# shendurelab/MIPGEN

Measured on AMD Instinct MI355X. Metric: candidate MIPs scored/sec (SVR), higher is better.
Workload: dtype f64

## Files before the change

### mipgen_amd/csrc/kernels_svr.hip

```cpp
#include <hip/hip_runtime.h>
#include "kernels.h"
#include "device_utils.h"
#include "exp2_coef.h"
#include "mip_record.h"
#include <stdlib.h>

namespace {

__device__ __forceinline__ void exp2x3(double& t0, double& t1, double& t2)
{
    constexpr double C[11] = EXP2_COEF_10;
    const double MAGIC = 6755399441055744.0;
    double m0, m1, m2, f0, f1, f2;
    const double cd = C[10];
    asm volatile(
        "v_add_f64 %[m0], %[t0], %[magic]\n\t"
        "v_add_f64 %[m1], %[t1], %[magic]\n\t"
        "v_add_f64 %[m2], %[t2], %[magic]\n\t"
        "v_add_f64 %[f0], %[m0], -%[magic]\n\t"
        "v_add_f64 %[f1], %[m1], -%[magic]\n\t"
        "v_add_f64 %[f2], %[m2], -%[magic]\n\t"
        "v_add_f64 %[f0], %[t0], -%[f0]\n\t"
        "v_add_f64 %[f1], %[t1], -%[f1]\n\t"
        "v_add_f64 %[f2], %[t2], -%[f2]\n\t"
        "v_fma_f64 %[t0], %[cd], %[f0], %[c9]\n\t"
        "v_fma_f64 %[t1], %[cd], %[f1], %[c9]\n\t"
        "v_fma_f64 %[t2], %[cd], %[f2], %[c9]\n\t"
        "v_fma_f64 %[t0], %[t0], %[f0], %[c8]\n\t"
        "v_fma_f64 %[t1], %[t1], %[f1], %[c8]\n\t"
        "v_fma_f64 %[t2], %[t2], %[f2], %[c8]\n\t"
        "v_fma_f64 %[t0], %[t0], %[f0], %[c7]\n\t"
        "v_fma_f64 %[t1], %[t1], %[f1], %[c7]\n\t"
        "v_fma_f64 %[t2], %[t2], %[f2], %[c7]\n\t"
        "v_fma_f64 %[t0], %[t0], %[f0], %[c6]\n\t"
        "v_fma_f64 %[t1], %[t1], %[f1], %[c6]\n\t"
        "v_fma_f64 %[t2], %[t2], %[f2], %[c6]\n\t"
        "v_fma_f64 %[t0], %[t0], %[f0], %[c5]\n\t"
        "v_fma_f64 %[t1], %[t1], %[f1], %[c5]\n\t"
        "v_fma_f64 %[t2], %[t2], %[f2], %[c5]\n\t"
        "v_fma_f64 %[t0], %[t0], %[f0], %[c4]\n\t"
        "v_fma_f64 %[t1], %[t1], %[f1], %[c4]\n\t"
        "v_fma_f64 %[t2], %[t2], %[f2], %[c4]\n\t"
        "v_fma_f64 %[t0], %[t0], %[f0], %[c3]\n\t"
        "v_fma_f64 %[t1], %[t1], %[f1], %[c3]\n\t"
        "v_fma_f64 %[t2], %[t2], %[f2], %[c3]\n\t"
        "v_fma_f64 %[t0], %[t0], %[f0], %[c2]\n\t"
        "v_fma_f64 %[t1], %[t1], %[f1], %[c2]\n\t"
        "v_fma_f64 %[t2], %[t2], %[f2], %[c2]\n\t"
        "v_fma_f64 %[t0], %[t0], %[f0], %[c1]\n\t"
        "v_fma_f64 %[t1], %[t1], %[f1], %[c1]\n\t"
        "v_fma_f64 %[t2], %[t2], %[f2], %[c1]\n\t"
        "v_fma_f64 %[t0], %[t0], %[f0], %[c0]\n\t"
        "v_fma_f64 %[t1], %[t1], %[f1], %[c0]\n\t"
        "v_fma_f64 %[t2], %[t2], %[f2], %[c0]\n\t"
        : [t0] "+v"(t0), [t1] "+v"(t1), [t2] "+v"(t2), [m0] "=&v"(m0), [m1] "=&v"(m1), [m2] "=&v"(m2),
          [f0] "=&v"(f0), [f1] "=&v"(f1), [f2] "=&v"(f2)
        : [cd] "v"(cd), [magic] "s"(MAGIC), [c0] "s"(C[0]), [c1] "s"(C[1]), [c2] "s"(C[2]), [c3] "s"(C[3]), [c4] "s"(C[4]),
          [c5] "s"(C[5]), [c6] "s"(C[6]), [c7] "s"(C[7]), [c8] "s"(C[8]), [c9] "s"(C[9]));
    t0 = __hiloint2double(__double2hiint(t0) + (__double2loint(m0) << 20), __double2loint(t0));
    t1 = __hiloint2double(__double2hiint(t1) + (__double2loint(m1) << 20), __double2loint(t1));
    t2 = __hiloint2double(__double2hiint(t2) + (__double2loint(m2) << 20), __double2loint(t2));
}

template <int N>
__device__ __forceinline__ double dpp_row_shr(double x)
{
    const int lo = __builtin_amdgcn_update_dpp(0, __double2loint(x), 0x110 | N, 0xf, 0xf, true);
    const int hi = __builtin_amdgcn_update_dpp(0, __double2hiint(x), 0x110 | N, 0xf, 0xf, true);
    return __hiloint2double(hi, lo);
}
__device__ __forceinline__ double readlane_f64(double x, int l)
{
    return __hiloint2double(__builtin_amdgcn_readlane(__double2hiint(x), l), __builtin_amdgcn_readlane(__double2loint(x), l));
}

__device__ __forceinline__ int arm_feat(int base, int idx) { return base + idx + (idx >= 15); }
__device__ __forceinline__ int ins_feat(int idx) { return F_INS + idx + (idx >= 63); }

}

extern "C" int mipgen_svr_scores_fit_lds(int np, int kc, int n_pairs, int ss_range, int ssmax, int Lmax, int n_arm, int group, int n_e, int n_l, int n_threads, int it_pitch)
{
    const SvrLayout La = svr_layout(np, ssmax - ss_range + 1, ssmax, Lmax, n_arm, group, n_e, n_l, n_threads, it_pitch);
    const SvrLayout Lb = svr_layout(np, ssmax - ss_range + 1, ssmax, Lmax, n_arm, group, n_l, n_e, n_threads, it_pitch);
    const int need = np * kc * n_pairs;
    return need <= La.total_bytes / 8 - La.pf && need <= Lb.total_bytes / 8 - Lb.pf;
}

extern "C" size_t mipgen_svr_lds_bytes_tile(int np, int ss_range, int ssmax, int Lmax, int n_arm, int group, int n_e, int n_l, int n_threads, int it_pitch)
{
    const SvrLayout La = svr_layout(np, ssmax - ss_range + 1, ssmax, Lmax, n_arm, group, n_e, n_l, n_threads, it_pitch);
    const SvrLayout Lb = svr_layout(np, ssmax - ss_range + 1, ssmax, Lmax, n_arm, group, n_l, n_e, n_threads, it_pitch);
    if ((size_t)La.tb_stride * group * 8 > 65535 || (size_t)Lb.tb_stride * group * 8 > 65535) return (size_t)1 << 30;
    const size_t a = (size_t)La.total_bytes, b = (size_t)Lb.total_bytes;
    return a > b ? a : b;
}

__device__ __forceinline__ void svr_steps2(double& a0, double& a1, uint32_t lu, uint32_t ld, uint32_t pg0, uint32_t pg1,
                                           double i00, double i01, double i02, double i10, double i11, double i12)
{
    double u00, u01, u02, d00, d01, d02, u10, u11, u12, d10, d11, d12;
    uint32_t au0, ad0, au1, ad1, s0, s1, s2, s3;
    asm volatile(
        "s_and_b32 %[s0], %[pg0], 0xffff\n\t"
        "s_lshr_b32 %[s1], %[pg0], 16\n\t"
        "s_and_b32 %[s2], %[pg1], 0xffff\n\t"
        "s_lshr_b32 %[s3], %[pg1], 16\n\t"
        "v_add_u32 %[au0], %[s0], %[lu]\n\t"
        "v_add_u32 %[ad0], %[s1], %[ld]\n\t"
        "v_add_u32 %[au1], %[s2], %[lu]\n\t"
        "v_add_u32 %[ad1], %[s3], %[ld]\n\t"
        "ds_read_b64 %[u00], %[au0]\n\t"
        "ds_read_b64 %[d00], %[ad0]\n\t"
        "ds_read_b64 %[u01], %[au0] offset:8\n\t"
        "ds_read_b64 %[d01], %[ad0] offset:8\n\t"
        "ds_read_b64 %[u02], %[au0] offset:16\n\t"
        "ds_read_b64 %[d02], %[ad0] offset:16\n\t"
        "ds_read_b64 %[u10], %[au1]\n\t"
        "ds_read_b64 %[d10], %[ad1]\n\t"
        "ds_read_b64 %[u11], %[au1] offset:8\n\t"
        "ds_read_b64 %[d11], %[ad1] offset:8\n\t"
        "ds_read_b64 %[u12], %[au1] offset:16\n\t"
        "ds_read_b64 %[d12], %[ad1] offset:16\n\t"
        "s_waitcnt lgkmcnt(10)\n\t"
        "v_mul_f64 %[u00], %[u00], %[d00]\n\t"
        "s_waitcnt lgkmcnt(8)\n\t"
        "v_mul_f64 %[u01], %[u01], %[d01]\n\t"
        "v_fma_f64 %[a0], %[i00], %[u00], %[a0]\n\t"
        "s_waitcnt lgkmcnt(6)\n\t"
        "v_mul_f64 %[u02], %[u02], %[d02]\n\t"
        "v_fma_f64 %[a0], %[i01], %[u01], %[a0]\n\t"
        "s_waitcnt lgkmcnt(4)\n\t"
        "v_mul_f64 %[u10], %[u10], %[d10]\n\t"
        "v_fma_f64 %[a0], %[i02], %[u02], %[a0]\n\t"
        "s_waitcnt lgkmcnt(2)\n\t"
        "v_mul_f64 %[u11], %[u11], %[d11]\n\t"
        "v_fma_f64 %[a1], %[i10], %[u10], %[a1]\n\t"
        "s_waitcnt lgkmcnt(0)\n\t"
        "v_mul_f64 %[u12], %[u12], %[d12]\n\t"
        "v_fma_f64 %[a1], %[i11], %[u11], %[a1]\n\t"
        "v_fma_f64 %[a1], %[i12], %[u12], %[a1]\n\t"
        : [a0] "+v"(a0), [a1] "+v"(a1), [u00] "=&v"(u00), [u01] "=&v"(u01), [u02] "=&v"(u02), [d00] "=&v"(d00), [d01] "=&v"(d01),
          [d02] "=&v"(d02), [u10] "=&v"(u10), [u11] "=&v"(u11), [u12] "=&v"(u12), [d10] "=&v"(d10), [d11] "=&v"(d11), [d12] "=&v"(d12),
          [au0] "=&v"(au0), [ad0] "=&v"(ad0), [au1] "=&v"(au1), [ad1] "=&v"(ad1), [s0] "=&s"(s0), [s1] "=&s"(s1), [s2] "=&s"(s2), [s3] "=&s"(s3)
        : [lu] "v"(lu), [ld] "v"(ld), [pg0] "s"(pg0), [pg1] "s"(pg1), [i00] "v"(i00), [i01] "v"(i01), [i02] "v"(i02),
          [i10] "v"(i10), [i11] "v"(i11), [i12] "v"(i12)
        : "memory", "scc");
}
__device__ __forceinline__ void svr_steps1(double& a0, uint32_t lu, uint32_t ld, uint32_t pg0, double i00, double i01, double i02)
{
    double u00, u01, u02, d00, d01, d02;
    uint32_t au0, ad0, s0, s1;
    asm volatile(
        "s_and_b32 %[s0], %[pg0], 0xffff\n\t"
        "s_lshr_b32 %[s1], %[pg0], 16\n\t"
        "v_add_u32 %[au0], %[s0], %[lu]\n\t"
        "v_add_u32 %[ad0], %[s1], %[ld]\n\t"
        "ds_read_b64 %[u00], %[au0]\n\t"
        "ds_read_b64 %[d00], %[ad0]\n\t"
        "ds_read_b64 %[u01], %[au0] offset:8\n\t"
        "ds_read_b64 %[d01], %[ad0] offset:8\n\t"
        "ds_read_b64 %[u02], %[au0] offset:16\n\t"
        "ds_read_b64 %[d02], %[ad0] offset:16\n\t"
        "s_waitcnt lgkmcnt(4)\n\t"
        "v_mul_f64 %[u00], %[u00], %[d00]\n\t"
        "s_waitcnt lgkmcnt(2)\n\t"
        "v_mul_f64 %[u01], %[u01], %[d01]\n\t"
        "v_fma_f64 %[a0], %[i00], %[u00], %[a0]\n\t"
        "s_waitcnt lgkmcnt(0)\n\t"
        "v_mul_f64 %[u02], %[u02], %[d02]\n\t"
        "v_fma_f64 %[a0], %[i01], %[u01], %[a0]\n\t"
        "v_fma_f64 %[a0], %[i02], %[u02], %[a0]\n\t"
        : [a0] "+v"(a0), [u00] "=&v"(u00), [u01] "=&v"(u01), [u02] "=&v"(u02), [d00] "=&v"(d00), [d01] "=&v"(d01), [d02] "=&v"(d02),
          [au0] "=&v"(au0), [ad0] "=&v"(ad0), [s0] "=&s"(s0), [s1] "=&s"(s1)
        : [lu] "v"(lu), [ld] "v"(ld), [pg0] "s"(pg0), [i00] "v"(i00), [i01] "v"(i01), [i02] "v"(i02)
        : "memory", "scc");
}

template <int C>
__device__ __forceinline__ void svr_scan_rows(const __attribute__((address_space(3))) uint32_t* tab,
                                              const __attribute__((address_space(3))) double* sv,
                                              __attribute__((address_space(3))) double* out, bool act, double c2)
{
    typedef __attribute__((address_space(3))) const char lds_cc;
    typedef __attribute__((address_space(3))) const double lds_cd;
    lds_cc* svb = (lds_cc*)sv;
    double v[C];
    double tot = 0.0;
#pragma unroll
    for (int q = 0; q < C; q += 4) {
        uint32_t t[4];
        double g[4];
#pragma unroll
        for (int j = 0; j < 4; j++) if (q + j < C) t[j] = tab[q + j];
#pragma unroll
        for (int j = 0; j < 4; j++) if (q + j < C) g[j] = *(lds_cd*)(svb + t[j]);
#pragma unroll
        for (int j = 0; j < 4; j++) if (q + j < C) { v[q + j] = tot; tot = fma(g[j], c2, tot); }
    }
    double x = tot;
    x += dpp_row_shr<1>(x); x += dpp_row_shr<2>(x); x += dpp_row_shr<4>(x); x += dpp_row_shr<8>(x);
    const double base = x - tot;
    if (act) {
#pragma unroll
        for (int q = 0; q < C; q++) out[q * SVR_GROUP] = base + v[q];
    }
}

struct ScanDesc {
    int o0;
    int k;
    int ax, ay;
    int thr;
    int base;
    int len;
    int out;
    int ixo;
    int c;
    int blk;
    int pad[5];
};

#ifndef SVR_MIN_WAVES
#define SVR_MIN_WAVES 3
#endif
template <int CL>
__global__ __launch_bounds__(SVR_MAX_THREADS, 4) void k_svr_dense(
    const DevParams* __restrict__ P, const SvrGeom G, const DevRegion* __restrict__ regions,
    const SvrTile* __restrict__ tiles, int n_tiles, const uint8_t* __restrict__ bases,
    const int32_t* __restrict__ copy, const double* __restrict__ log10_tab, const double* __restrict__ model_all, int n_sv_all,
    double gamma_l2e, double rho, double s_guard, const uint64_t* __restrict__ records, double* __restrict__ scores,
    int n_split, double* __restrict__ partials, int64_t part_stride
#ifdef MIPGEN_DIAG
    , int dbg, unsigned long long* __restrict__ prof
#endif
    )
{
#ifndef MIPGEN_DIAG
    constexpr int dbg = 0;
    unsigned long long* const prof = nullptr;
#endif
    extern __shared__ __align__(16) unsigned char smem[];
    const unsigned long long blk_enter = ((dbg & 8) && prof) ? __builtin_amdgcn_s_memrealtime() : 0;
    const int unit = blockIdx.x;
    const int tile_i = unit / n_split, part = unit - tile_i * n_split;
    const SvrTile tile = tiles[tile_i];
    const DevRegion& R = regions[tile.region];
    const int groups_all = (n_sv_all + SVR_GROUP - 1) / SVR_GROUP, gpp = (groups_all + n_split - 1) / n_split;
    const int sv0 = part * gpp * SVR_GROUP;
    const double* __restrict__ model = model_all + (int64_t)sv0 * SV_ROW;
    const int n_sv = max(0, min(n_sv_all - sv0, gpp * SVR_GROUP));
    const int tid = threadIdx.x, lane = tid & (WAVE - 1);
    const int wid = __builtin_amdgcn_readfirstlane(tid / WAVE);
    const int NT = blockDim.x, NW = NT / WAVE;
    const bool minus = tile.strand != 0;

    const int A = P->n_pairs;
    const int Lmax = max(P->e_max, P->l_max);
    const int n_arm = max(G.n_e, G.n_l) | 1;
    const int Cmax_t = P->max_capture - (R.k0 + tile.ki0) * P->inc;
    const int Cmin_t = Cmax_t - (tile.kc - 1) * P->inc;
    const int ssmax = Cmax_t - P->min_sum, ssmin = Cmin_t - P->max_sum;
    const int p_first = R.first_pos + tile.p0;
    const int lo = p_first - Lmax;
    const int up_min = minus ? +P->l_min : +P->e_min;
    const int dn_min = minus ? +P->e_min : +P->l_min;
    const int n_up = minus ? +G.n_l : +G.n_e, n_dn = minus ? +G.n_e : +G.n_l;
    const int up_base = minus ? F_LIG : F_EXT, dn_base = minus ? F_EXT : F_LIG;
    const int up_len_f = minus ? F_LIG_LEN : F_EXT_LEN, dn_len_f = minus ? F_EXT_LEN : F_LIG_LEN;
    const int up_cp_f = minus ? F_LLC : F_LEC, dn_cp_f = minus ? F_LEC : F_LLC;
    const int up_norm_f = minus ? SVR_N_LIG : SVR_N_EXT, dn_norm_f = minus ? SVR_N_EXT : SVR_N_LIG;

    const SvrLayout L = svr_layout(tile.np, ssmin, ssmax, Lmax, n_arm, SVR_GROUP, n_up, n_dn, (int)blockDim.x, tile.pad >> 8);
    int L_ku = L.ku, L_kd = L.kd, L_tu = L.tu, L_td = L.td, L_ins = L.ins_len, L_up = L.up_cnt, L_dn = L.dn_cnt;
    asm volatile("" : "+s"(L_ku), "+s"(L_kd), "+s"(L_tu), "+s"(L_td), "+s"(L_ins), "+s"(L_up), "+s"(L_dn));
    const int S_ins = __builtin_amdgcn_readfirstlane(L.ins_sl), S_up = __builtin_amdgcn_readfirstlane(L.up_sl), S_dn = __builtin_amdgcn_readfirstlane(L.dn_sl);
    double* const dbase = (double*)smem;
    double* rinv = dbase + L.rinv;
    double* lg10 = dbase + L.lg10;
    uint32_t* ent_a = (uint32_t*)(smem + L.bytes_ent);
    uint32_t* ent_b = ent_a + L.n_ent_lds;
    const double cneg = -gamma_l2e, c2 = 2.0 * gamma_l2e;
    uint16_t* psum = (uint16_t*)(smem + L.bytes_psum);
    uint32_t* work = (uint32_t*)(smem + L.bytes_psum + 2 * SVR_MAX_CHUNK * (SVR_MAX_THREADS / 64));
    double* rows = dbase + L.rows;
    double* pfb = dbase + L.pf;
    double* tbb = dbase + L.tb;
    double* itb = dbase + L.it;
    ScanDesc* desc = (ScanDesc*)(smem + L.bytes_desc);
    uint32_t* sidx = (uint32_t*)(smem + L.bytes_idx);
    uint8_t* sb = smem + L.bytes_sb;
    const int ssr = ssmax - ssmin + 1;
    const int nq_t = L.nq;

    for (int i = tid; i < L.span_b + 8; i += NT) {
        int ri = lo + i - R.seq_start;
        sb[i] = (i < L.span_b && ri >= 0 && ri < R.seq_len) ? (bases[R.seq_off + ri] & BASE_CODE_MASK) : (uint8_t)BASE_OTHER;
    }
    for (int i = tid; i < L.rinv_len; i += NT) {
        rinv[3 * i] = i > 0 ? 1.0 / (double)i : 0.0; rinv[3 * i + 1] = i > 1 ? 1.0 / (double)(i - 1) : 0.0;
        rinv[3 * i + 2] = i > 2 ? 1.0 / (double)(i - 2) : 0.0;
    }
    for (int i = tid; i < 102; i += NT) lg10[i] = i == 0 ? 0.0 : (i <= 100 ? log10_tab[i] : 2.0);
    for (int i = tid; i < MIPGEN_N_LRC; i += NT) lg10[102 + i] = R.lrc[i];
    for (int i = tid; i < A && i < SVR_MAX_CHUNK * (SVR_MAX_THREADS / 64); i += NT) psum[i] = (uint16_t)((P->arm_ext[i] + P->arm_lig[i]) * L.it_p);
    if (tid < SVR_N_ARR) {
        ScanDesc d;
        const int k = tid;
        const bool ins = k < 3, up = k == 3 || k == 4;
        d.o0 = ins ? Lmax : (up ? 0 : Lmax + ssmin);
        d.k = ins ? k + 1 : ((k - 3) & 1) + 1;
        d.ax = ins ? 21 : 5; d.ay = ins ? 5 : 1; d.thr = ins ? 63 : 15;
        d.base = ins ? F_INS : (up ? up_base : dn_base);
        d.len = ins ? L_ins : (up ? L_up : L_dn);
        d.out = (ins ? k : 3) * S_ins + (ins ? 0 : (up ? k - 3 : 2)) * S_up + (k < 5 ? 0 : k - 5) * S_dn;
        d.ixo = d.out; d.c = (ins ? +S_ins : (up ? +S_up : +S_dn)) / 16;
        d.blk = ins ? 1 : ((up ? minus : !minus) ? 2 : 0);
        desc[k] = d;
    }
    __syncthreads();

    for (int k = 0; k < SVR_N_ARR; k++) {
        const ScanDesc d = desc[k];
        for (int i = tid; i < 16 * d.c; i += NT) {
            int slot = SVR_ZERO;
            if (i < d.len) {
                const int b0 = sb[d.o0 + i], b1 = sb[d.o0 + i + 1], b2 = sb[d.o0 + i + 2];
                const int last = d.k == 1 ? b0 : (d.k == 2 ? b1 : b2);
                const bool ok = b0 < 4 && (d.k < 2 || b1 < 4) && (d.k < 3 || b2 < 4);
                const int x = minus ? 3 - last : b0;
                const int y = d.k == 2 ? (minus ? 3 - b0 : b1) : (minus ? 3 - b1 : b1);
                const int z = minus ? 3 - b0 : b2;
                const int idx = d.ax * x + (d.k >= 2 ? d.ay * y + 1 : 0) + (d.k == 3 ? z + 1 : 0);
                if (ok) slot = d.k == 1 ? SVR_C1 + 4 * d.blk + x
                                        : d.base + idx + (idx >= d.thr);
            }
            sidx[d.ixo + i] = (uint32_t)(slot * (SVR_GROUP * 8));
        }
    }

    const int nU = tile.np * n_up, nD = nq_t * n_dn, n_ent = nU + nD;
    auto arm_entry = [&](int w, uint32_t& e_a, uint32_t& e_b, double* norm) __attribute__((always_inline)) {
        const bool up = w < nU;
        int wl, li, len, s;
        if (up) { wl = w / n_up; li = w - wl * n_up; len = up_min + li; s = Lmax + wl - len; }
        else { const int w2 = w - nU; wl = w2 / n_dn; li = w2 - wl * n_dn; len = dn_min + li; s = Lmax + ssmin + wl; }
        const bool is_lig = up ? minus : !minus;
        (void)norm;
        int cp = 1;
        if (R.copy_off >= 0) {
            const int slot = P->len_slot[len];
            const int ri = lo + s - R.seq_start;
            cp = (slot >= 0 && ri >= 0 && ri < R.seq_len) ? copy[R.copy_off + (int64_t)slot * R.seq_len + ri] : 0;
        }
        const uint32_t cpc = (uint32_t)min(max(cp, 0), 101);
        uint32_t jcode = 0;
        if (is_lig) {
            int j0, j1;
            if (!minus) { j0 = sb[s]; j1 = sb[s + 1]; }
            else { j0 = comp_code(sb[s + len - 1]); j1 = comp_code(sb[s + len - 2]); }
            jcode = (j0 < 4 && j1 < 4) ? (uint32_t)(4 * j0 + j1 + 1) : 17u;
        }
        const int s0 = up ? s : wl;
        e_a = (uint32_t)((3 * S_ins + (up ? 0 : 2 * S_up) + s0) * (SVR_GROUP * 8)) | ((uint32_t)(((up ? L_tu : L_td) + wl * n_arm + li) * (SVR_GROUP * 8)) << 16);
        e_b = (uint32_t)len | ((uint32_t)up << 7) | ((jcode * (SVR_GROUP * 8)) << 8) | ((cpc * 8) << 17);
    };
    for (int w = tid; w < n_ent; w += NT) { uint32_t ea_, eb_; arm_entry(w, ea_, eb_, nullptr); ent_a[w] = ea_; ent_b[w] = eb_; }

    const int chunk = wid / G.wpc;
    const int item = (wid - chunk * G.wpc) * WAVE + lane;
    const int np_lane = svr_np_lane(tile.np, tile.kc, P->inc, G.wpc * WAVE);
    const int kci_l = item / np_lane, pl_l = item - kci_l * np_lane;
    const bool owner = chunk < G.nchunk && kci_l < tile.kc && pl_l < tile.np;
    const int kci = owner ? kci_l : 0, pl = owner ? pl_l : 0;
    const int a_lo = min(chunk, G.nchunk - 1) * G.chunk_len;
    const int a_n = min(G.chunk_len, A - a_lo);
    const int C = Cmax_t - kci * P->inc;
    const uint32_t lane_u_off = (uint32_t)((L.tu + pl * n_arm) * (SVR_GROUP * 8));
    const int d_row = owner ? pl + C - P->max_sum - ssmin : svr_idle_d_row(item, np_lane, tile.kc, P->inc, nq_t, P->max_sum - P->min_sum);
    const uint32_t lane_d_off = (uint32_t)((L.td + d_row * n_arm) * (SVR_GROUP * 8));
    const int prog0 = __builtin_amdgcn_readfirstlane((minus ? MIPGEN_MAX_ARM_PAIRS + 16 : 0) + a_lo);
    uint32_t newS_v = 0;
#pragma unroll
    for (int i = 0; i < CL; i++) {
        const int a = a_lo + min(i, a_n - 1);
        if (i == 0 || (i < a_n && P->arm_ext[a - 1] + P->arm_lig[a - 1] != P->arm_ext[a] + P->arm_lig[a])) newS_v |= 1u << i;
    }
    const uint32_t newS = __builtin_amdgcn_readfirstlane(newS_v);
    const int it_pl = owner ? pl : svr_idle_it_col(item, L.it_p, np_lane, tile.kc, P->inc);
    const int iB = ((C - ssmin) * L.it_p + it_pl) * SVR_GROUP;
    double acc[CL];
#pragma unroll
    for (int i = 0; i < CL; i++) acc[i] = 0.0;
    const bool wave_owns = __builtin_amdgcn_ballot_w64(owner) != 0;

    if (tid == 0) {
        int* kp = (int*)(smem + L.bytes_kpar);
        kp[0] = nU; kp[1] = n_up; kp[2] = n_dn; kp[3] = up_min; kp[4] = dn_min; kp[5] = Lmax; kp[6] = ssmin; kp[7] = n_ent;
        kp[8] = L_tu; kp[9] = L_td; kp[10] = n_arm; kp[11] = tile.np; kp[12] = ssmax; kp[13] = L.it_p; kp[14] = minus ? 1 : 0;
    }

    const int n_groups = (n_sv + SVR_GROUP - 1) / SVR_GROUP;
    constexpr int ROW_N = SVR_GROUP * SV_ROW;
    constexpr int ROW_R = 1;
    const int64_t row_lim = (int64_t)n_sv * SV_ROW;
    auto row_fetch = [&](int k, int j) -> double {
        const int64_t gk = (int64_t)k * ROW_N + j;
        return (j < ROW_N && gk < row_lim) ? model[gk] : 0.0;
    };
    auto row_slot = [&](int k, int j) -> int { const int g = j / SV_ROW; return (k & 1) * ROW_N + (j - g * SV_ROW) * SVR_GROUP + g; };
    auto load_rows_direct = [&](int k) __attribute__((always_inline)) { for (int j = tid; j < ROW_N; j += NT) rows[row_slot(k, j)] = row_fetch(k, j); };

    typedef __attribute__((address_space(3))) const double lds_cd;
    typedef volatile __attribute__((address_space(3))) const double lds_vcd;
    typedef __attribute__((address_space(3))) double lds_d;
    typedef __attribute__((address_space(3))) const uint32_t lds_cu;
    constexpr int S_UNITS = 7;
    auto stage_scan = [&](int k) __attribute__((always_inline)) {
        lds_cd* rowk = (lds_cd*)rows + (k & 1) * ROW_N;
        lds_d* PF = (lds_d*)pfb + (k & 1) * SVR_GROUP * L.pf_stride;
        for (int u = wid; u < S_UNITS + 1; u += NW) {
            if (u < S_UNITS) {
                const int cls = u < 3 ? 0 : (u < 5 ? 1 : 2);
                const int r = (u - (cls == 0 ? 0 : (cls == 1 ? 3 : 5))) * 4 + (lane >> 4);
                const bool act = r < (cls == 0 ? 3 : 2) * SVR_GROUP;
                const int rr = act ? r : 0;
                const int arr_in = rr / SVR_GROUP, g = rr - arr_in * SVR_GROUP;
                const int sl = S_ins + (cls >= 1) * (S_up - S_ins) + (cls >= 2) * (S_dn - S_up);
                const int c = sl >> 4;
                const int first = (cls >= 1) * 3 * S_ins + (cls >= 2) * 2 * S_up + arr_in * sl + (lane & 15) * c;
                lds_cu* tab = (lds_cu*)sidx + first;
                lds_cd* sv = rowk + g;
                lds_d* out = PF + first * SVR_GROUP + g;
                if (c == 5) svr_scan_rows<5>(tab, sv, out, act, c2);
                else if (c == 7) svr_scan_rows<7>(tab, sv, out, act, c2);
                else if (c == 9) svr_scan_rows<9>(tab, sv, out, act, c2);
                else if (c == 11) svr_scan_rows<11>(tab, sv, out, act, c2);
                else if (c == 13) svr_scan_rows<13>(tab, sv, out, act, c2);
                else if (c == 3) svr_scan_rows<3>(tab, sv, out, act, c2);
                else {
                    double tot = 0.0;
                    for (int j = 0; j < c; j++) tot = fma(sv[tab[j] >> 3], c2, tot);
                    double x = tot;
                    x += dpp_row_shr<1>(x); x += dpp_row_shr<2>(x); x += dpp_row_shr<4>(x); x += dpp_row_shr<8>(x);
                    double run = x - tot;
                    for (int j = 0; j < c; j++) {
                        if (act) out[j * SVR_GROUP] = run;
                        run = fma(sv[tab[j] >> 3], c2, run);
                    }
                }
            } else {
                const bool up_half = lane < 32;
                const int hl = up_half ? lane : lane - 32;
                const bool have_len = up_half ? hl < n_up : hl < n_dn;
                const int f_len = up_half ? up_len_f : dn_len_f, f_norm = up_half ? up_norm_f : dn_norm_f;
                const bool junc = up_half ? minus : !minus;
                const int lrc_i = lane < MIPGEN_N_LRC ? lane : 0, tj_i = (lane >= 1 && lane <= 16) ? lane - 1 : 0;
                double v_len[SVR_GROUP], v_norm[SVR_GROUP], v_junc[SVR_GROUP], v_lrc[SVR_GROUP], v_nins[SVR_GROUP], v_nextra[SVR_GROUP], v_tj[SVR_GROUP], v_ilen[SVR_GROUP];
                const double lrc_x = ((lds_cd*)lg10)[102 + lrc_i];
#pragma unroll
                for (int g = 0; g < SVR_GROUP; g++) {
                    lds_cd* sv = rowk + g;
                    v_len[g] = sv[f_len * SVR_GROUP]; v_norm[g] = sv[f_norm * SVR_GROUP]; v_junc[g] = sv[SVR_N_JUNC * SVR_GROUP];
                    v_lrc[g] = sv[(F_LRC + lrc_i) * SVR_GROUP]; v_nins[g] = sv[SVR_N_INS * SVR_GROUP]; v_nextra[g] = sv[SVR_N_EXTRA * SVR_GROUP];
                    v_tj[g] = sv[(F_JUNC + tj_i) * SVR_GROUP]; v_ilen[g] = sv[F_INS_LEN * SVR_GROUP];
                }
                double dlr[SVR_GROUP];
#pragma unroll
                for (int g = 0; g < SVR_GROUP; g++) {
                    const double dl = (double)((up_half ? up_min : dn_min) + hl) - v_len[g];
                    if (have_len) PF[((up_half ? L.ku : L.kd) + hl) * SVR_GROUP + g] = cneg * (v_norm[g] + dl * dl + (junc ? v_junc[g] : 0.0));
                    const double d = lrc_x - v_lrc[g];
                    dlr[g] = lane < MIPGEN_N_LRC ? d * d : 0.0;
                }
#pragma unroll
                for (int g = 0; g < SVR_GROUP; g++) dlr[g] += dpp_row_shr<1>(dlr[g]);
#pragma unroll
                for (int g = 0; g < SVR_GROUP; g++) dlr[g] += dpp_row_shr<2>(dlr[g]);
#pragma unroll
                for (int g = 0; g < SVR_GROUP; g++) dlr[g] += dpp_row_shr<4>(dlr[g]);
#pragma unroll
                for (int g = 0; g < SVR_GROUP; g++) dlr[g] += dpp_row_shr<8>(dlr[g]);
#pragma unroll
                for (int g = 0; g < SVR_GROUP; g++) {
                    const double tot = (readlane_f64(dlr[g], 15) + readlane_f64(dlr[g], 31)) + (readlane_f64(dlr[g], 47) + readlane_f64(dlr[g], 63));
                    const double ci = cneg * (tot + v_nins[g] + v_nextra[g]);
                    if (lane == 0) PF[L.ci * SVR_GROUP + g] = ci;
                    if (lane < 18) PF[(L.tj + lane) * SVR_GROUP + g] = (lane >= 1 && lane <= 16) ? fma(v_tj[g], c2, cneg) : 0.0;
                    const double sl = v_ilen[g];
                    for (int j = lane; j < ssr; j += WAVE) { const double dl = (double)(ssmin + j) - sl; PF[(L.ti + j) * SVR_GROUP + g] = fma(dl * cneg, dl, ci); }
                }
            }
        }
    };

    const int n_ins = tile.np * ssr;
    const int n_ent_pad = (n_ent + WAVE - 1) & ~(WAVE - 1), n_tot = n_ent_pad + n_ins;
    const int lane_q = lane / ssr, lane_r = lane - lane_q * ssr;
    typedef volatile __attribute__((address_space(3))) const uint32_t lds_vcu;
    auto lds_addr = [](const void* p) -> uint32_t { return (uint32_t)(__UINTPTR_TYPE__)(const __attribute__((address_space(3))) char*)p; };
    const uint32_t rows_a = lds_addr(rows), pf_a0 = lds_addr(pfb), tb_a = lds_addr(tbb), it_a = lds_addr(itb), rv_a = lds_addr(rinv), lg_a = lds_addr(lg10);
    const uint32_t ea_a = lds_addr(ent_a), eb_a = lds_addr(ent_b);
    const uint32_t pf_bytes = (uint32_t)(SVR_GROUP * L.pf_stride * 8);
    constexpr uint32_t SLOT = SVR_GROUP * 8;
    const uint32_t dBu = (uint32_t)(L.up_sl * SLOT - SLOT), dBd = (uint32_t)(L.dn_sl * SLOT - SLOT);
    const uint32_t kU = (uint32_t)((L_ku - up_min) * SLOT), kD = (uint32_t)((L_kd - dn_min) * SLOT);
    const uint32_t scU = (uint32_t)(up_cp_f * SLOT), scD = (uint32_t)(dn_cp_f * SLOT);
    const uint32_t tj_off = (uint32_t)(L.tj * SLOT), ti_off = (uint32_t)(L.ti * SLOT);
    const uint32_t i1 = (uint32_t)(L.ins_sl * SLOT);
    const uint32_t ss0 = (uint32_t)(ssmin * SLOT);
    auto ldp = [](uint32_t a) -> lds_vcd* { return (lds_vcd*)(unsigned long)a; };
    auto stage_tables = [&](int k) __attribute__((always_inline)) {
        const uint32_t rowk_a = rows_a + (uint32_t)((k & 1) * ROW_N * 8);
        const uint32_t PF_a = pf_a0 + (uint32_t)(k & 1) * pf_bytes;
        for (;;) {
            __builtin_amdgcn_s_setprio(2);
            uint32_t b0 = 0;
            if (lane == 0) b0 = __hip_atomic_fetch_add(work, (uint32_t)WAVE, __ATOMIC_RELAXED, __HIP_MEMORY_SCOPE_WORKGROUP);
            const int base = (int)__builtin_amdgcn_readfirstlane(b0);
            if (base >= n_tot) break;
            const int w = base + lane;
            if (w >= n_tot || (base < n_ent_pad && w >= n_ent)) continue;
            double x[SVR_GROUP];
            uint32_t dst;
            if (base < n_ent_pad) {
                const uint32_t ea = *(lds_vcu*)(unsigned long)(ea_a + ((uint32_t)w << 2)), eb = *(lds_vcu*)(unsigned long)(eb_a + ((uint32_t)w << 2));
                const uint32_t len = eb & 127u;
                const bool is_up = (eb & 128u) != 0;
                const uint32_t A1 = PF_a + (ea & 0xFFFFu);
                const uint32_t lenS = __umul24(len, SLOT);
                const uint32_t A0 = A1 + lenS;
                const uint32_t Bp = A1 + (is_up ? dBu : dBd);
                const uint32_t B0 = Bp + lenS;
                const uint32_t Kp = PF_a + (is_up ? kU : kD) + lenS;
                const uint32_t Tj = PF_a + tj_off + ((eb >> 8) & 0x1FFu);
                const uint32_t Sc = rowk_a + (is_up ? scU : scD);
                lds_vcd* rv = ldp(rv_a + __umul24(len, 24u));
                const double r1 = rv[0], r2 = rv[1];
                const double lc = *ldp(lg_a + ((eb >> 17) & 0x3FFu));
                double a0[SVR_GROUP], a1[SVR_GROUP], q0[SVR_GROUP], q1[SVR_GROUP], kp[SVR_GROUP], tj[SVR_GROUP], sc[SVR_GROUP];
#pragma unroll
                for (int g = 0; g < SVR_GROUP; g++) { a0[g] = ldp(A0)[g]; a1[g] = ldp(A1)[g]; q0[g] = ldp(B0)[g]; q1[g] = ldp(Bp)[SVR_GROUP + g]; kp[g] = ldp(Kp)[g]; tj[g] = ldp(Tj)[g]; sc[g] = ldp(Sc)[g]; }
                __builtin_amdgcn_s_setprio(0);
#pragma unroll
                for (int g = 0; g < SVR_GROUP; g++) {
                    const double dc = lc - sc[g];
                    double t = kp[g] + tj[g];
                    t = fma(a0[g] - a1[g], r1, t);
                    t = fma(q0[g] - q1[g], r2, t);
                    t = fma(dc * cneg, dc, t);
                    x[g] = fmax(t, -330.0);
                }
                exp2x3(x[0], x[1], x[2]);
                dst = tb_a + (ea >> 16);
            } else {
                const int bq = (base - n_ent_pad) / ssr, br = (base - n_ent_pad) - bq * ssr;
                int ssi = br + lane_r, pi = bq + lane_q;
                if (ssi >= ssr) { ssi -= ssr; pi++; }
                const uint32_t ssiS = __umul24((uint32_t)ssi, SLOT);
                const uint32_t F1 = PF_a + __umul24((uint32_t)pi, SLOT);
                const uint32_t E1 = F1 + ss0 + ssiS;
                const uint32_t F2 = F1 + i1, F3 = F2 + i1;
                const uint32_t E2 = E1 + (i1 - SLOT), E3 = E1 + (2u * i1 - 2u * SLOT);
                const uint32_t Ti = PF_a + ti_off + ssiS;
                lds_vcd* rv = ldp(rv_a + __umul24((uint32_t)(ssmin + ssi), 24u));
                const double r0 = rv[0], r1 = rv[1], r2 = rv[2];
                lds_vcd* Cf = ldp(rowk_a + SVR_COEF * SLOT);
                double f1a[SVR_GROUP], f1b[SVR_GROUP], f2a[SVR_GROUP], f2b[SVR_GROUP], f3a[SVR_GROUP], f3b[SVR_GROUP], ti[SVR_GROUP], cf[SVR_GROUP];
#pragma unroll
                for (int g = 0; g < SVR_GROUP; g++) { f1a[g] = ldp(E1)[g]; f1b[g] = ldp(F1)[g]; f2a[g] = ldp(E2)[g]; f2b[g] = ldp(F2)[g]; f3a[g] = ldp(E3)[g]; f3b[g] = ldp(F3)[g]; ti[g] = ldp(Ti)[g]; cf[g] = Cf[g]; }
                __builtin_amdgcn_s_setprio(0);
#pragma unroll
                for (int g = 0; g < SVR_GROUP; g++) {
                    double t = ti[g];
                    t = fma(f1a[g] - f1b[g], r0, t);
                    t = fma(f2a[g] - f2b[g], r1, t);
                    t = fma(f3a[g] - f3b[g], r2, t);
                    x[g] = fmax(t, -330.0);
                }
                exp2x3(x[0], x[1], x[2]);
#pragma unroll
                for (int g = 0; g < SVR_GROUP; g++) x[g] *= cf[g];
                dst = it_a + __umul24((uint32_t)(__mul24(ssi, L.it_p) + pi), SLOT);
            }
            lds_d* dstp = (lds_d*)(unsigned long)dst;
#pragma unroll
            for (int g = 0; g < SVR_GROUP; g++) dstp[g] = x[g];
        }
    };

    load_rows_direct(0); load_rows_direct(1);
    if (tid == 0) *work = 0u;
    __syncthreads();
    if (!(dbg & 1)) stage_scan(0);
    __syncthreads();

    unsigned long long blk_t0 = 0; unsigned hwid = 0, xcc = 0;
    if ((dbg & 8) && prof) { blk_t0 = __builtin_amdgcn_s_memrealtime(); asm volatile("s_getreg_b32 %0, hwreg(HW_REG_HW_ID)" : "=s"(hwid)); asm volatile("s_getreg_b32 %0, hwreg(HW_REG_XCC_ID)" : "=s"(xcc)); }
    unsigned long long pc[6] = {0, 0, 0, 0, 0, 0};
    const bool stamp = (dbg & 8) && prof;
    typedef volatile __attribute__((address_space(3))) double lds_vd;
    const lds_vd* tb3 = (const lds_vd*)tbb;
    const lds_vd* it3 = (const lds_vd*)itb;
    const uint32_t tba = (uint32_t)(__UINTPTR_TYPE__)tb3;

    for (int i = 0; i < n_groups; i++) {
        const unsigned long long t0 = stamp ? __builtin_readcyclecounter() : 0;
        __builtin_amdgcn_s_setprio(1);
        if (i + 1 < n_groups && !(dbg & 1)) stage_scan(i + 1);
        __builtin_amdgcn_s_setprio(0);
        const unsigned long long t1 = stamp ? __builtin_readcyclecounter() : 0;
        if (!(dbg & 2)) stage_tables(i);
        __builtin_amdgcn_s_setprio(0);
        const unsigned long long t2 = stamp ? __builtin_readcyclecounter() : 0;
        __syncthreads();
        const unsigned long long t3 = stamp ? __builtin_readcyclecounter() : 0;
        if (tid == 0) *work = 0u;
        double rowreg[ROW_R];
#pragma unroll
        for (int r = 0; r < ROW_R; r++) rowreg[r] = row_fetch(i + 2, tid + r * NT);
        if (!(dbg & 4) && wave_owns) {
            static_assert(SVR_GROUP == 3, "three staged support vectors per step");
            double I0 = 0.0, I1 = 0.0, I2 = 0.0;
            uint32_t sum = psum[a_lo];
            uint32_t ns = newS;
            const uint32_t lane_u = tba + lane_u_off, lane_d = tba + lane_d_off;
            int pgi = prog0;
            asm volatile("" : "+s"(pgi));
            uint32_t pg[CL];
#pragma unroll
            for (int q = 0; q < CL; q++) pg[q] = (&P->pair_prog[0][0])[pgi + q];
            asm volatile("" : "+s"(ns));
#pragma unroll
            for (int ii = 0; ii < CL; ii += 2) {
                if (ii == 0) __builtin_amdgcn_s_setprio(3); else if (ii == (CL / 4 + 1) / 2 * 2) __builtin_amdgcn_s_setprio(2);
                else if (ii == (CL / 2 + 1) / 2 * 2) __builtin_amdgcn_s_setprio(1); else if (ii == (3 * CL / 4 + 1) / 2 * 2) __builtin_amdgcn_s_setprio(0);
                if (ns & (1u << ii)) {
                    const lds_vd* ip = it3 + (iB - __mul24((int)sum, SVR_GROUP));
                    I0 = ip[0]; I1 = ip[1]; I2 = ip[2];
                    const uint32_t later = ns >> (ii + 1);
                    if (later) sum = psum[a_lo + ii + 1 + __builtin_ctz(later)];
                }
                const double A0 = I0, A1 = I1, A2 = I2;
                if (ii + 1 < CL) {
                    if (ns & (1u << (ii + 1))) {
                        const lds_vd* ip = it3 + (iB - __mul24((int)sum, SVR_GROUP));
                        I0 = ip[0]; I1 = ip[1]; I2 = ip[2];
                        const uint32_t later = ii + 2 < 32 ? ns >> (ii + 2) : 0u;
                        if (later) sum = psum[a_lo + ii + 2 + __builtin_ctz(later)];
                    }
                    svr_steps2(acc[ii], acc[ii + 1 < CL ? ii + 1 : 0], lane_u, lane_d, pg[ii], pg[ii + 1 < CL ? ii + 1 : 0], A0, A1, A2, I0, I1, I2);
                } else {
                    svr_steps1(acc[ii], lane_u, lane_d, pg[ii], A0, A1, A2);
                }
            }
        }
        __builtin_amdgcn_s_setprio(0);
        const unsigned long long t4 = stamp ? __builtin_readcyclecounter() : 0;
#pragma unroll
        for (int r = 0; r < ROW_R; r++) { const int j = tid + r * NT; if (j < ROW_N) rows[row_slot(i, j)] = rowreg[r]; }
        for (int j = tid + ROW_R * NT; j < ROW_N; j += NT) rows[row_slot(i, j)] = row_fetch(i + 2, j);
        const unsigned long long t5 = stamp ? __builtin_readcyclecounter() : 0;
        __syncthreads();
        if (stamp) { const unsigned long long t6 = __builtin_readcyclecounter(); pc[0] += t1 - t0; pc[1] += t2 - t1; pc[2] += t4 - t3; pc[3] += t3 - t2; pc[4] += t6 - t0; pc[5] += t6 - t5; }
    }
    if (stamp && lane == 0 && blockIdx.x >= 400 && blockIdx.x < 432 && wid < 16) for (int k = 0; k < 6; k++) prof[((blockIdx.x - 400) * 16 + wid) * 6 + k] = pc[k];
    if (stamp && tid == 0 && blockIdx.x < 4096) { unsigned long long* q = prof + 64 * 8 * 6 + (size_t)blockIdx.x * 8; q[0] = hwid; q[1] = xcc; q[2] = blk_t0; q[3] = __builtin_amdgcn_s_memrealtime(); q[4] = blk_enter; q[6] = ((unsigned long long)tile.np << 32) | (unsigned)tile.kc; q[7] = ((unsigned long long)n_ent << 32) | (unsigned)(tile.np * ssr); }

    {
        volatile const int* kp = (volatile const int*)(smem + L.bytes_kpar);
        const int k_nU = __builtin_amdgcn_readfirstlane(kp[0]), k_nup = __builtin_amdgcn_readfirstlane(kp[1]), k_ndn = __builtin_amdgcn_readfirstlane(kp[2]);
        const int k_upmin = __builtin_amdgcn_readfirstlane(kp[3]), k_dnmin = __builtin_amdgcn_readfirstlane(kp[4]), k_Lmax = __builtin_amdgcn_readfirstlane(kp[5]);
        const int k_ssmin = __builtin_amdgcn_readfirstlane(kp[6]), k_nent = __builtin_amdgcn_readfirstlane(kp[7]), k_tu = __builtin_amdgcn_readfirstlane(kp[8]);
        const int k_td = __builtin_amdgcn_readfirstlane(kp[9]), k_narm = __builtin_amdgcn_readfirstlane(kp[10]), k_np = __builtin_amdgcn_readfirstlane(kp[11]);
        const int k_ssmax = __builtin_amdgcn_readfirstlane(kp[12]), k_itp = __builtin_amdgcn_readfirstlane(kp[13]), k_minus = __builtin_amdgcn_readfirstlane(kp[14]);
        const double kneg = -gamma_l2e;
        constexpr double CE[11] = EXP2_COEF_10;
        auto exp2_one = [&](double t) -> double {
            t = fmax(t, -1000.0);
            const double MAGIC = 6755399441055744.0;
            const double m = t + MAGIC;
            const double f = t - (m - MAGIC);
            double pp = CE[10];
#pragma unroll
            for (int k = 9; k >= 0; k--) pp = fma(pp, f, CE[k]);
            return __hiloint2double(__double2hiint(pp) + (__double2loint(m) << 20), __double2loint(pp));
        };
        uint32_t* cnt = (uint32_t*)pfb;
        int* insq = (int*)(cnt + 80 * k_np);
        const int k_ssr = k_ssmax - k_ssmin + 1;
        const int e1_waves = NW > 1 ? max(1, min((2 * k_np + WAVE - 1) / WAVE, NW / 2)) : 1;
        if (wid < e1_waves) {
            for (int pli = tid >> 1; pli < k_np; pli += e1_waves * (WAVE / 2)) {
                const int lvl = tid & 1;
                uint32_t* c = cnt + pli * 80 + (lvl ? 16 : 0);
                for (int k = 0; k < (lvl ? 64 : 16); k++) c[k] = 0;
                uint64_t c1p = 0;
                int q = 0, b1 = BASE_OTHER, b2 = BASE_OTHER;
                const int s0 = k_Lmax + pli;
                for (int n = 1; n <= k_ssmax; n++) {
                    const int bb = sb[s0 + n - 1];
                    if (bb < 4) {
                        c1p += 1ull << (16 * bb);
                        if (b1 < 4 && (!lvl || b2 < 4)) {
                            const int d = lvl ? 16 * b2 + 4 * b1 + bb : 4 * b1 + bb;
                            q += 2 * (int)atomicAdd(&c[d], 1u) + 1;
                        }
                    }
                    b2 = b1; b1 = bb;
                    if (n >= k_ssmin) {
                        int* o = insq + (pli * k_ssr + (n - k_ssmin)) * 4;
                        if (lvl) o[3] = q;
                        else {
                            const int c1[4] = {(int)(c1p & 0xFFFF), (int)((c1p >> 16) & 0xFFFF), (int)((c1p >> 32) & 0xFFFF), (int)(c1p >> 48)};
                            o[0] = c1[0] * c1[0] + c1[1] * c1[1] + c1[2] * c1[2] + c1[3] * c1[3]; o[1] = q; o[2] = c1[BASE_C] + c1[BASE_G];
                        }
                    }
                }
            }
        }
        if (wid >= e1_waves || NW == 1) {
            const int arm_t0 = NW == 1 ? tid : tid - e1_waves * WAVE, arm_nt = NW == 1 ? NT : NT - e1_waves * WAVE;
            for (int w = arm_t0; w < k_nent; w += arm_nt) {
                const bool up = w < k_nU;
                int wl, li, len, st;
                if (up) { wl = w / k_nup; li = w - wl * k_nup; len = k_upmin + li; st = k_Lmax + wl - len; }
                else { const int w2 = w - k_nU; wl = w2 / k_ndn; li = w2 - wl * k_ndn; len = k_dnmin + li; st = k_Lmax + k_ssmin + wl; }
                uint64_t clo = 0, chi = 0;
                uint64_t c1p = 0;
                int prev = BASE_OTHER;
                for (int i = 0; i < len; i++) {
                    const int b = sb[st + i];
                    if (b < 4) {
                        c1p += 1ull << (16 * b);
                        if (prev < 4) {
                            const int d = 4 * prev + b;
                            if (d & 8) chi += 1ull << ((d & 7) * 8); else clo += 1ull << ((d & 7) * 8);
                        }
                    }
                    prev = b;
                }
                int q2 = 0;
#pragma unroll
                for (int k = 0; k < 8; k++) {
                    const int a = (int)((clo >> (8 * k)) & 0xFF), b = (int)((chi >> (8 * k)) & 0xFF);
                    q2 += a * a + b * b;
                }
                const int c1[4] = {(int)(c1p & 0xFFFF), (int)((c1p >> 16) & 0xFFFF), (int)((c1p >> 32) & 0xFFFF), (int)(c1p >> 48)};
                const int q1 = c1[0] * c1[0] + c1[1] * c1[1] + c1[2] * c1[2] + c1[3] * c1[3];
                const double dl = (double)len, dl1 = (double)(len - 1);
                const double gc = (double)(c1[BASE_C] + c1[BASE_G]) / dl;
                tbb[((up ? k_tu : k_td) + wl * k_narm + li) * SVR_GROUP] = exp2_one(kneg * ((double)q1 / (dl * dl) + (double)q2 / (dl1 * dl1) + gc * gc));
            }
        }
        __syncthreads();
        for (int e = tid; e < k_np * k_ssr; e += NT) {
            const int pli = e / k_ssr, j = e - pli * k_ssr, n = k_ssmin + j;
            const int* o = insq + e * 4;
            const double dn = (double)n, dn1 = (double)(n - 1), dn2 = (double)(n - 2);
            const double gc = (double)o[2] / dn;
            itb[(j * k_itp + pli) * SVR_GROUP] = exp2_one(kneg * ((double)o[0] / (dn * dn) + (double)o[1] / (dn1 * dn1) + (double)o[3] / (dn2 * dn2) + gc * gc));
        }
        __syncthreads();
        if (owner) {
            const char* tbc = (const char*)tbb;
#pragma unroll
            for (int i = 0; i < CL; i++) {
                if (i < a_n) {
                    const uint32_t pgw = P->pair_prog[k_minus][a_lo + i];
                    const double fu = *(const double*)(tbc + lane_u_off + (pgw & 0xffffu)), fd = *(const double*)(tbc + lane_d_off + (pgw >> 16));
                    const double fi = itb[iB - (int)psum[a_lo + i] * SVR_GROUP];
                    acc[i] *= fu * fd * fi;
                }
            }
        }
    }

    {
        const int n_items = tile.np * tile.kc;
        const int nK = R.n_sizes;
        if (tile.pad & 1) {
            double* const stg = dbase + L.pf;
            __syncthreads();
            if (owner) {
                const int item_own = kci * tile.np + pl;
#pragma unroll
                for (int i = 0; i < CL; i++) if (i < a_n) stg[item_own * A + a_lo + i] = acc[i];
            }
            __syncthreads();
            constexpr int WB = 4;
            for (int e0 = tid; e0 < n_items * A; e0 += WB * NT) {
                int64_t idx[WB];
                uint64_t rec[WB];
                double v[WB];
#pragma unroll
                for (int k = 0; k < WB; k++) {
                    const int e = min(e0 + k * NT, n_items * A - 1);
                    const int it_ = e / A, a = e - it_ * A;
                    const int kc_ = it_ / tile.np, pl_ = it_ - kc_ * tile.np;
                    idx[k] = R.out_off + ((((int64_t)(tile.p0 + pl_) * nK + (tile.ki0 + kc_)) * 2 + (minus ? 1 : 0)) * A) + a;
                    v[k] = stg[e];
                    rec[k] = n_split > 1 ? 0ull : records[idx[k]];
                }
#pragma unroll
                for (int k = 0; k < WB; k++) {
                    if (e0 + k * NT >= n_items * A) break;
                    if (n_split > 1) {
                        if (part == 0) scores[idx[k]] = v[k]; else partials[(int64_t)(part - 1) * part_stride + idx[k]] = v[k];
                        continue;
                    }
                    const double sc = record_score(rec[k], v[k] - rho, rho, s_guard);
#ifndef SVR_NO_STORE
                    scores[idx[k]] = sc;
#else
                    if (sc == 123.456) scores[idx[k]] = sc;
#endif
                }
            }
            if (stamp && tid == 0 && blockIdx.x < 4096) { __builtin_amdgcn_s_waitcnt(0); prof[64 * 8 * 6 + (size_t)blockIdx.x * 8 + 5] = __builtin_amdgcn_s_memrealtime(); }
            return;
        }
    }
    if (owner) {
        const int nK = R.n_sizes;
        const int64_t row0 = R.out_off + ((((int64_t)(tile.p0 + pl) * nK + (tile.ki0 + kci)) * 2 + (minus ? 1 : 0)) * A);
#pragma unroll
        for (int i = 0; i < CL; i++) {
            if (i < a_n) {
                const int64_t idx = row0 + (a_lo + i);
                if (n_split > 1) {
                    if (part == 0) scores[idx] = acc[i]; else partials[(int64_t)(part - 1) * part_stride + idx] = acc[i];
                    continue;
                }
                scores[idx] = record_score(records[idx], acc[i] - rho, rho, s_guard);
            }
        }
    }
}

__global__ __launch_bounds__(256) void k_svr_finish(int64_t n, int n_split, const double* __restrict__ partials, int64_t part_stride,
                                                    const uint64_t* __restrict__ records, double rho, double s_guard, double* __restrict__ scores)
{
    for (int64_t idx = (int64_t)blockIdx.x * blockDim.x + threadIdx.x; idx < n; idx += (int64_t)gridDim.x * blockDim.x) {
        double s = scores[idx];
        for (int k = 1; k < n_split; k++) s += partials[(int64_t)(k - 1) * part_stride + idx];
        scores[idx] = record_score(records[idx], s - rho, rho, s_guard);
    }
}

#ifdef MIPGEN_DIAG
static unsigned long long* g_prof = nullptr;
static int g_dbg = 0;
extern "C" void mipgen_svr_debug_set(int dbg) { g_dbg = dbg; }
extern "C" int mipgen_svr_debug_dump(unsigned long long* host, int n)
{
    if (!g_prof || n > 64 * 8 * 6 + 4096 * 8) return -1;
    if (hipDeviceSynchronize() != hipSuccess) return -2;
    return hipMemcpy(host, g_prof, (size_t)n * sizeof(unsigned long long), hipMemcpyDeviceToHost) == hipSuccess ? 0 : -3;
}
#endif

extern "C" hipError_t mipgen_launch_svr_dense(
    hipStream_t stream, int n_tiles, int n_tiles_few, size_t lds_bytes, const DevParams* P, const SvrGeom* G_main, const SvrGeom* G_few, const DevRegion* regions,
    const SvrTile* tiles, const uint8_t* bases, const int32_t* copy, const double* log10_tab, const double* model, int n_sv,
    double gamma_l2e, double rho, double s_guard, const uint64_t* records, double* scores, int64_t n_cand, int n_split, double* partials)
{
    if (n_tiles + n_tiles_few <= 0) return hipSuccess;
    if (n_split < 1 || (n_split > 1 && !partials)) return hipErrorInvalidValue;
#ifdef MIPGEN_DIAG
    const int dbg = g_dbg;
    if ((dbg & 8) && !g_prof) { if (hipMalloc((void**)&g_prof, (64 * 8 * 6 + 4096 * 8) * sizeof(unsigned long long)) != hipSuccess) g_prof = nullptr; }
    unsigned long long* prof = g_prof;
#define DIAG_ARGS , dbg, prof
#else
#define DIAG_ARGS
#endif
#define LAUNCH(C)                                                                                                          \
    do {                                                                                                                 \
        hipError_t e_ = hipFuncSetAttribute((const void*)k_svr_dense<C>, hipFuncAttributeMaxDynamicSharedMemorySize,        \
                                            (int)lds_bytes);                                                             \
        if (e_ != hipSuccess) return e_;                                                                                 \
        hipLaunchKernelGGL((k_svr_dense<C>), dim3(nt * n_split), dim3(G->nchunk * G->wpc * 64), lds_bytes, stream, P, *G, regions, tl, \
                           nt, bases, copy, log10_tab, model, n_sv, gamma_l2e, rho, s_guard, records, scores, n_split,   \
                           partials, n_cand DIAG_ARGS);                                                                  \
    } while (0)
    for (int pass = 0; pass < 2; pass++) {
        const SvrGeom* G = pass == 0 ? G_main : G_few;
        const SvrTile* tl = pass == 0 ? tiles : tiles + n_tiles;
        const int nt = pass == 0 ? n_tiles : n_tiles_few;
        if (nt <= 0) continue;
        if (G->chunk_len <= 5) LAUNCH(5);
        else if (G->chunk_len <= 8) LAUNCH(8);
        else if (G->chunk_len <= 10) LAUNCH(10);
        else if (G->chunk_len <= 15) LAUNCH(15);
        else return hipErrorInvalidValue;
        hipError_t e = hipGetLastError();
        if (e != hipSuccess) return e;
    }
#undef LAUNCH
#undef DIAG_ARGS
    if (n_split == 1) return hipSuccess;
    const int blocks = (int)((n_cand + 255) / 256 < 65536 ? (n_cand + 255) / 256 : 65536);
    hipLaunchKernelGGL(k_svr_finish, dim3(blocks), dim3(256), 0, stream, n_cand, n_split, partials, n_cand, records, rho, s_guard, scores);
    return hipGetLastError();
}
```

Baseline: 1.816 billion.

## Split k-mer insert stats into per-order wave jobs with batched unrolled loads

Rewrites the per-position insert statistics precompute so that each wave handles one k-mer order (1, 2 or 3) for a run of 64 consecutive positions, one position per lane. This replaces the old scheme where lane pairs shared a position and branched on level. Sequence bytes are loaded in unrolled batches of 8, and the k-mer index is kept as a rolling shifted value. The atomic adds are issued unconditionally with an add of 0 when no count is needed, so the divergent branches go away. The change aims to cut divergence and serial latency in this phase. In exchange it issues extra atomics, and it may read past k_ssmax when the batch rounds up.

```diff
diff --git a/mipgen_amd/csrc/kernels_svr.hip b/mipgen_amd/csrc/kernels_svr.hip
--- a/mipgen_amd/csrc/kernels_svr.hip
+++ b/mipgen_amd/csrc/kernels_svr.hip
@@ -686,34 +686,58 @@
             for (int k = 9; k >= 0; k--) pp = fma(pp, f, CE[k]);
             return __hiloint2double(__double2hiint(pp) + (__double2loint(m) << 20), __double2loint(pp));
         };
+        constexpr int NB = 8;
         uint32_t* cnt = (uint32_t*)pfb;
         int* insq = (int*)(cnt + 80 * k_np);
         const int k_ssr = k_ssmax - k_ssmin + 1;
-        const int e1_waves = NW > 1 ? max(1, min((2 * k_np + WAVE - 1) / WAVE, NW / 2)) : 1;
+        const int n_jobs = 3 * ((k_np + WAVE - 1) / WAVE);
+        const int e1_waves = NW > 1 ? max(1, min(n_jobs, NW / 2)) : 1;
         if (wid < e1_waves) {
-            for (int pli = tid >> 1; pli < k_np; pli += e1_waves * (WAVE / 2)) {
-                const int lvl = tid & 1;
-                uint32_t* c = cnt + pli * 80 + (lvl ? 16 : 0);
-                for (int k = 0; k < (lvl ? 64 : 16); k++) c[k] = 0;
-                uint64_t c1p = 0;
-                int q = 0, b1 = BASE_OTHER, b2 = BASE_OTHER;
-                const int s0 = k_Lmax + pli;
-                for (int n = 1; n <= k_ssmax; n++) {
-                    const int bb = sb[s0 + n - 1];
-                    if (bb < 4) {
-                        c1p += 1ull << (16 * bb);
-                        if (b1 < 4 && (!lvl || b2 < 4)) {
-                            const int d = lvl ? 16 * b2 + 4 * b1 + bb : 4 * b1 + bb;
-                            q += 2 * (int)atomicAdd(&c[d], 1u) + 1;
+            for (int job = wid; job < n_jobs; job += e1_waves) {
+                const int kk = job % 3 + 1, pli = (job / 3) * WAVE + lane;
+                if (pli >= k_np) continue;
+                const uint8_t* s = sb + k_Lmax + pli;
+                int* o = insq + pli * k_ssr * 4;
+                if (kk == 1) {
+                    uint64_t c1p = 0;
+                    for (int n0 = 0; n0 < k_ssmax; n0 += NB) {
+                        int bb[NB];
+#pragma unroll
+                        for (int k = 0; k < NB; k++) bb[k] = s[n0 + k];
+#pragma unroll
+                        for (int k = 0; k < NB; k++) {
+                            const int n = n0 + k + 1;
+                            if (bb[k] < 4) c1p += 1ull << (16 * bb[k]);
+                            if (n >= k_ssmin && n <= k_ssmax) {
+                                const int c1[4] = {(int)(c1p & 0xFFFF), (int)((c1p >> 16) & 0xFFFF), (int)((c1p >> 32) & 0xFFFF), (int)(c1p >> 48)};
+                                o[(n - k_ssmin) * 4] = c1[0] * c1[0] + c1[1] * c1[1] + c1[2] * c1[2] + c1[3] * c1[3];
+                                o[(n - k_ssmin) * 4 + 2] = c1[BASE_C] + c1[BASE_G];
+                            }
                         }
                     }
-                    b2 = b1; b1 = bb;
-                    if (n >= k_ssmin) {
-                        int* o = insq + (pli * k_ssr + (n - k_ssmin)) * 4;
-                        if (lvl) o[3] = q;
-                        else {
-                            const int c1[4] = {(int)(c1p & 0xFFFF), (int)((c1p >> 16) & 0xFFFF), (int)((c1p >> 32) & 0xFFFF), (int)(c1p >> 48)};
-                            o[0] = c1[0] * c1[0] + c1[1] * c1[1] + c1[2] * c1[2] + c1[3] * c1[3]; o[1] = q; o[2] = c1[BASE_C] + c1[BASE_G];
+                } else {
+                    uint32_t* c = cnt + pli * 80 + (kk == 3 ? 16 : 0);
+                    for (int k = 0; k < (kk == 3 ? 32 : 8); k++) ((uint64_t*)c)[k] = 0;
+                    const uint32_t mask = kk == 3 ? 63u : 15u;
+                    uint32_t idx = 0;
+                    int run = 0, q = 0;
+                    o += kk == 3 ? 3 : 1;
+                    for (int n0 = 0; n0 < k_ssmax; n0 += NB) {
+                        uint32_t bb[NB], add[NB], old[NB];
+#pragma unroll
+                        for (int k = 0; k < NB; k++) bb[k] = s[n0 + k];
+#pragma unroll
+                        for (int k = 0; k < NB; k++) {
+                            run = bb[k] < 4 ? run + 1 : 0;
+                            idx = ((idx << 2) | (bb[k] & 3u)) & mask;
+                            add[k] = (run >= kk && n0 + k < k_ssmax) ? 1u : 0u;
+                            old[k] = atomicAdd(&c[idx], add[k]);
+                        }
+#pragma unroll
+                        for (int k = 0; k < NB; k++) {
+                            const int n = n0 + k + 1;
+                            q += (int)(add[k] * (2u * old[k] + 1u));
+                            if (n >= k_ssmin && n <= k_ssmax) o[(n - k_ssmin) * 4] = q;
                         }
                     }
                 }
```

New measurement: 1.823 billion (median of 6 runs). About the same (+0.4%).
